# facebookresearch/D3GA

Measured on AMD Instinct MI355X. Metric: fwd+bwd frames/sec @500k Gaussians 1920x1080, higher is better.
Workload: dtype f32

## Files before the change

d3ga_amd/csrc/raster_composite_scan.hip:

```cpp
#include "composite_common.h"

#ifndef D3GA_SCAN_ABL
#define D3GA_SCAN_ABL 0
#endif
#ifndef D3GA_TILE_WAVES
#define D3GA_TILE_WAVES 4
#endif
#ifndef D3GA_TILE_PRIO
#define D3GA_TILE_PRIO 0
#endif

namespace d3ga {

#define D3GA_SCAN4(OP, BC, N) \
    OP " %0, %0, %0 row_shr:" #N " row_mask:0xf bank_mask:0xf" BC "\n" \
    OP " %1, %1, %1 row_shr:" #N " row_mask:0xf bank_mask:0xf" BC "\n" \
    OP " %2, %2, %2 row_shr:" #N " row_mask:0xf bank_mask:0xf" BC "\n" \
    OP " %3, %3, %3 row_shr:" #N " row_mask:0xf bank_mask:0xf" BC "\n"
#define D3GA_SCANX(OP, CTRL, MASK) \
    OP " %0, %0, %0 " CTRL " row_mask:" MASK " bank_mask:0xf\n" \
    OP " %1, %1, %1 " CTRL " row_mask:" MASK " bank_mask:0xf\n" \
    OP " %2, %2, %2 " CTRL " row_mask:" MASK " bank_mask:0xf\n" \
    OP " %3, %3, %3 " CTRL " row_mask:" MASK " bank_mask:0xf\n"
template <int R = 1>
__device__ __forceinline__ void row_scan_mul4(float &a, float &b, float &c, float &d) {
    asm("s_nop 1\n" D3GA_SCAN4("v_mul_f32_dpp", "", 1) D3GA_SCAN4("v_mul_f32_dpp", "", 2) D3GA_SCAN4("v_mul_f32_dpp", "", 4)
        D3GA_SCAN4("v_mul_f32_dpp", "", 8)
        : "+v"(a), "+v"(b), "+v"(c), "+v"(d));
    if constexpr (R >= 2) asm("s_nop 1\n" D3GA_SCANX("v_mul_f32_dpp", "row_bcast:15", "0xa") : "+v"(a), "+v"(b), "+v"(c), "+v"(d));
    if constexpr (R >= 4) asm("s_nop 1\n" D3GA_SCANX("v_mul_f32_dpp", "row_bcast:31", "0xc") : "+v"(a), "+v"(b), "+v"(c), "+v"(d));
}
template <int R = 1>
__device__ __forceinline__ void row_scan_add4(float &a, float &b, float &c, float &d) {
    asm("s_nop 1\n" D3GA_SCAN4("v_add_f32_dpp", " bound_ctrl:1", 1) D3GA_SCAN4("v_add_f32_dpp", " bound_ctrl:1", 2)
        D3GA_SCAN4("v_add_f32_dpp", " bound_ctrl:1", 4) D3GA_SCAN4("v_add_f32_dpp", " bound_ctrl:1", 8)
        : "+v"(a), "+v"(b), "+v"(c), "+v"(d));
    if constexpr (R >= 2) asm("s_nop 1\n" D3GA_SCANX("v_add_f32_dpp", "row_bcast:15", "0xa") : "+v"(a), "+v"(b), "+v"(c), "+v"(d));
    if constexpr (R >= 4) asm("s_nop 1\n" D3GA_SCANX("v_add_f32_dpp", "row_bcast:31", "0xc") : "+v"(a), "+v"(b), "+v"(c), "+v"(d));
}

struct ScanEntry {
    uint32_t pos, gid;
    float2 xy;
    float4 co;
    float4 rgb;
    float c2r, c2g, c2b;
};

template <bool DUAL>
__device__ __forceinline__ ScanEntry scan_gather(uint2 pg, const float2 *__restrict__ xy, const float4 *__restrict__ conic_o,
                                                 const float4 *__restrict__ rgb_invd, const float *__restrict__ colors2 ) {
    ScanEntry e;
    e.pos = pg.x; e.gid = pg.y;
    e.xy = make_float2(0.f, 0.f);
    e.co = make_float4(0.f, 0.f, 0.f, 0.f);
    e.rgb = make_float4(0.f, 0.f, 0.f, 0.f);
    e.c2r = e.c2g = e.c2b = 0.f;
    if (pg.x != 0u) {
        e.xy = xy[2 * (size_t)pg.y]; e.co = conic_o[pg.y]; e.rgb = rgb_invd[pg.y];
        if constexpr (DUAL) {
            e.c2r = colors2[3 * (size_t)pg.y]; e.c2g = colors2[3 * (size_t)pg.y + 1]; e.c2b = colors2[3 * (size_t)pg.y + 2];
        }
    }
    return e;
}

#ifdef D3GA_DIAG
__device__ unsigned long long g_diag_scan[16];
__device__ unsigned long long g_diag_waves[32768 * 4];
#endif
template <bool DUAL>
__device__ __forceinline__ void scan_consume(ScanEntry &e, uint2 &pg) {
    asm volatile("" : "+v"(e.xy.x), "+v"(e.xy.y), "+v"(e.co.x), "+v"(e.co.y), "+v"(e.co.z), "+v"(e.co.w));
    asm volatile("" : "+v"(e.rgb.x), "+v"(e.rgb.y), "+v"(e.rgb.z), "+v"(pg.x), "+v"(pg.y));
    if constexpr (DUAL) asm volatile("" : "+v"(e.c2r), "+v"(e.c2g), "+v"(e.c2b));
}

typedef float f4 __attribute__((ext_vector_type(4)));
typedef uint32_t u2 __attribute__((ext_vector_type(2)));
typedef __attribute__((address_space(3))) uint32_t lds_u32;

struct BwdArgs {
    int W, H, gx, gyv, P;
    const float2 *xy; const float4 *conic_o; const float4 *rgb_invd; const float *bg; const float *final_T; const uint32_t *n_contrib;
    const float *dL_dpix; float *acc; const float *colors2; const float *bg2; const float *dL_dpix2; const uint2 *blk_list;
    const uint32_t *blk_count; L1Source l1; const float *dL_dinvd;
    const int4 *win;
};
struct BwdDiag { unsigned long long install = 0, hit = 0, evict = 0, valid = 0, entries = 0, rowgroups = 0, trips = 0, groups = 0; };

template <bool DUAL, int S, bool INVD, int R, bool WIN>
__device__ __forceinline__ void bwd_tile_wave(const BwdArgs &A, const int tile, const uint32_t begin, const uint32_t end, const int blk,
                                              uint32_t *const s_cache, float *const s_pix, float *const s_dump, const int lane,
                                              BwdDiag &dg) {
    constexpr int PIXF = DUAL ? 12 : 8;
    constexpr int ROWF = 16 * PIXF + 4;
    constexpr int kSlot = 12;
    constexpr uint32_t kLocked = 0xffffffffu;
    constexpr int LW = 16 * R;
    const int row = lane / LW, l16 = lane & 15, lseg = lane & (LW - 1);
    constexpr int kVals = INVD ? 10 : 9, kPerInst = 64 / kVals;
    const int fq = lane / kVals, fk = lane - kVals * fq;
    const int fk_off = fk < 2 ? fk : fk + 1;
    constexpr int kAccStride = D3GA_ACC_STRIDE;
    const int bx = 2 * ((blk >> 2) & 1) + (blk & 1), by = 2 * (blk >> 3) + ((blk >> 1) & 1);
    const int tyb = tile / A.gx, view = tyb / A.gyv;
    int4 wv = make_int4(0, 0, A.W, A.H);
    if constexpr (WIN) wv = A.win[view];
    const int bx0 = (tile - tyb * A.gx) * kTile + 4 * bx + (WIN ? (wv.x & ~(kTile - 1)) : 0);
    const int by0 = (tyb - view * A.gyv) * kTile + 4 * by + (WIN ? (wv.y & ~(kTile - 1)) : 0);
    const int px = bx0 + (l16 & 3), py = by0 + (l16 >> 2);
    const bool inside = WIN ? (px >= wv.x && px < wv.x + A.W && py >= wv.y && py < wv.y + A.H) : (px < A.W && py < A.H);
    const int ix = WIN ? px - wv.x : px, iy = WIN ? py - wv.y : py;
    const size_t hw = (size_t)A.H * A.W;
    const size_t pid1 = hw * view + (size_t)iy * A.W + ix;
    const size_t pid = pid1 + 2 * hw * view;
    const float T_final = inside ? A.final_T[pid1] : 0.f;
    const uint32_t last = inside ? A.n_contrib[pid1] : 0u;
    float g0 = 0.f, g1 = 0.f, g2 = 0.f;
    if (inside && A.dL_dpix) { g0 = A.dL_dpix[pid]; g1 = A.dL_dpix[hw + pid]; g2 = A.dL_dpix[2 * hw + pid]; }
    if (inside && A.l1.image) {
        const float *tgt = A.l1.target_cell ? *A.l1.target_cell : A.l1.target;
        const float sc = A.l1.g_loss[0] * A.l1.inv_n;
        auto sgn = [](float d) { return d > 0.f ? 1.f : (d < 0.f ? -1.f : 0.f); };
        g0 += sc * sgn(A.l1.image[pid] - tgt[pid]);
        g1 += sc * sgn(A.l1.image[hw + pid] - tgt[hw + pid]);
        g2 += sc * sgn(A.l1.image[2 * hw + pid] - tgt[2 * hw + pid]);
    }
    float bg_dot = A.bg[0] * g0 + A.bg[1] * g1 + A.bg[2] * g2;
    float h0 = 0.f, h1 = 0.f, h2 = 0.f;
    if constexpr (DUAL) {
        if (inside) { h0 = A.dL_dpix2[pid]; h1 = A.dL_dpix2[hw + pid]; h2 = A.dL_dpix2[2 * hw + pid]; }
        bg_dot += A.bg2[0] * h0 + A.bg2[1] * h1 + A.bg2[2] * h2;
    }
    const uint32_t maxlast = wave_max_u32(last);
    if (maxlast == 0) return;

    float *const pixrow = s_pix + row * ROWF;
    float *const wr_base = lseg == LW - 1 ? pixrow : s_dump + 2 * lane;
    {
        float *rec = pixrow + l16 * PIXF;
        *reinterpret_cast<float4 *>(rec) = make_float4(T_final, 0.f, g0, g1);
        float gd = 0.f;
        if constexpr (INVD) gd = inside ? A.dL_dinvd[pid1] : 0.f;
        *reinterpret_cast<float4 *>(rec + 4) = make_float4(g2, T_final * bg_dot, __uint_as_float(last), gd);
        if constexpr (DUAL) *reinterpret_cast<float4 *>(rec + 8) = make_float4(h0, h1, h2, 0.f);
    }
    const uint32_t blk_cap = end - begin;
    const int qx0 = bx0 - 4 * (bx & 1), qy0 = by0 - 4 * (by & 1);
    const bool quad_in = WIN ? (qx0 < wv.x + A.W && qy0 < wv.y + A.H && qx0 + 8 > wv.x && qy0 + 8 > wv.y) : (qx0 < A.W && qy0 < A.H);
    const uint32_t cnt = quad_in ? A.blk_count[16 * (size_t)tile + blk] : 0u;
    const uint2 *const list = A.blk_list + 16 * (size_t)begin + (size_t)blk * blk_cap;
    const int ngroups = (int)((wave_max_u32(cnt) + (uint32_t)(LW - 1)) / (uint32_t)LW);
    const float ddelx_dx = 0.5f * (WIN ? wv.z : A.W), ddely_dy = 0.5f * (WIN ? wv.w : A.H);
    const float bxr = (float)bx0, byr = (float)by0;
    const int per = D3GA_SCAN_ABL == 12 ? LW : (ngroups > 0 ? ((int)cnt + ngroups - 1) / ngroups : 0);
    auto list_entry = [&](int g) -> uint2 {
        const int idx = (int)cnt - 1 - per * g - lseg;
        uint2 v = list[max(idx, 0)];
        v.x = (idx >= 0 && lseg < per) ? v.x : 0u;
        return v;
    };
    const float *const colors2v = DUAL ? A.colors2 - 3 * (size_t)view * (size_t)A.P : nullptr;
    ScanEntry e = scan_gather<DUAL>(list_entry(0), A.xy, A.conic_o, A.rgb_invd, colors2v);
    uint2 pg1 = list_entry(1);
    __builtin_amdgcn_wave_barrier();

    for (int g = 0; g < ngroups; ++g) {
        ScanEntry nxt = scan_gather<DUAL>(pg1, A.xy, A.conic_o, A.rgb_invd, colors2v);
        uint2 pg2 = list_entry(g + 2);
        const bool act = e.pos != 0u;
        const float exr = e.xy.x - bxr, eyr = e.xy.y - byr;
        const ConicQ cq = conic_q(e.co.x, e.co.y, e.co.z);
        float SA = 0.f, SB = 0.f, SC = 0.f, SyA = 0.f, SyB = 0.f, SyyA = 0.f, M6 = 0.f, M7 = 0.f, M8 = 0.f, M9 = 0.f;
#if D3GA_TILE_PRIO
        {
            const int left = ngroups - g;
            if (left > 8) __builtin_amdgcn_s_setprio(3);
            else if (left > 4) __builtin_amdgcn_s_setprio(2);
            else if (left > 2) __builtin_amdgcn_s_setprio(1);
            else __builtin_amdgcn_s_setprio(0);
        }
#endif
#pragma unroll 1
        for (int ky = 0; ky < (D3GA_SCAN_ABL == 8 ? 0 : 4); ++ky) {
            const float *const pixq = pixrow + ky * 4 * PIXF;
            float4 pa[4], pb[4], pc[4];
#pragma unroll
            for (int k = 0; k < 4; ++k) {
                pa[k] = *reinterpret_cast<const float4 *>(pixq + k * PIXF);
                pb[k] = *reinterpret_cast<const float4 *>(pixq + k * PIXF + 4);
                if constexpr (DUAL) pc[k] = *reinterpret_cast<const float4 *>(pixq + k * PIXF + 8);
                asm volatile("" : "+v"(pb[k].x), "+v"(pb[k].y), "+v"(pb[k].z));
                if constexpr (INVD) asm volatile("" : "+v"(pb[k].w));
            }
            const float dy = eyr - (float)ky;
            const float tb = cq.b * dy, tc = (cq.c * dy) * dy;
            float al[4], G[4], r[4], u[4], cgv[4], dx[4];
            bool valid[4];
#pragma unroll
            for (int k = 0; k < 4; ++k) {
                dx[k] = exr - (float)k;
                bool ok;
                splat_eval_q(dx[k], tb, tc, cq.a, e.co.w, al[k], G[k], ok);
                valid[k] = ok & (e.pos <= __float_as_uint(pb[k].z));
#ifdef D3GA_DIAG_COUNTERS
                dg.valid += valid[k] ? 1 : 0;
#endif
                al[k] = valid[k] ? al[k] : 0.f;
                r[k] = __builtin_amdgcn_rcpf(1.0f - al[k]);
                cgv[k] = e.rgb.x * pa[k].z + e.rgb.y * pa[k].w + e.rgb.z * pb[k].x;
                if constexpr (DUAL) cgv[k] += e.c2r * pc[k].x + e.c2g * pc[k].y + e.c2b * pc[k].z;
                if constexpr (INVD) cgv[k] = fmaf(e.rgb.w, pb[k].w, cgv[k]);
            }
            float p0 = r[0], p1 = r[1], p2 = r[2], p3 = r[3];
            row_scan_mul4<R>(p0, p1, p2, p3);
            const float Ti[4] = {pa[0].x * p0, pa[1].x * p1, pa[2].x * p2, pa[3].x * p3};
            float dch[4];
#pragma unroll
            for (int k = 0; k < 4; ++k) { dch[k] = al[k] * Ti[k]; u[k] = cgv[k] * dch[k]; }
            float s0 = u[0], s1 = u[1], s2 = u[2], s3 = u[3];
            row_scan_add4<R>(s0, s1, s2, s3);
            const float Sin[4] = {s0 + pa[0].y, s1 + pa[1].y, s2 + pa[2].y, s3 + pa[3].y};
            float *const wq = wr_base + ky * 4 * PIXF;
            float gop[4];
#pragma unroll
            for (int k = 0; k < 4; ++k) {
                const float dLda = Ti[k] * cgv[k] - (Sin[k] - u[k] + pb[k].y) * r[k];
                gop[k] = valid[k] ? G[k] * dLda : 0.f;
                M6 += dch[k] * pa[k].z; M7 += dch[k] * pa[k].w; M8 += dch[k] * pb[k].x;
                if constexpr (INVD) M9 = fmaf(dch[k], pb[k].w, M9);
                *reinterpret_cast<float2 *>(wq + k * PIXF) = make_float2(Ti[k], Sin[k]);
            }
            const float A = (gop[0] + gop[1]) + (gop[2] + gop[3]);
            const float B = fmaf(3.0f, gop[3], fmaf(2.0f, gop[2], gop[1]));
            const float C = fmaf(9.0f, gop[3], fmaf(4.0f, gop[2], gop[1]));
            SA += A; SB += B; SC += C;
            SyA = fmaf(dy, A, SyA); SyB = fmaf(dy, B, SyB); SyyA = fmaf(dy * dy, A, SyyA);
        }
        const float M5 = SA, ow = e.co.w;
        const float M0 = ow * (exr * SA - SB), M1 = ow * SyA;
        const float M2 = ow * (exr * (exr * SA - 2.0f * SB) + SC), M3 = ow * (exr * SyA - SyB), M4 = ow * SyyA;
        const float v0 = -(e.co.x * M0 + e.co.y * M1) * ddelx_dx;
        const float v1 = -(e.co.z * M1 + e.co.y * M0) * ddely_dy;
        const float4 va = make_float4(v0, v1, -0.5f * M2, -0.5f * M3), vb = make_float4(-0.5f * M4, M5, M6, M7);
        scan_consume<DUAL>(nxt, pg2);
        __builtin_amdgcn_wave_barrier();
        const uint32_t saddr = (uint32_t)(uintptr_t)(lds_u32 *)(s_cache + ((e.pos - 1u) & (uint32_t)(S - 1)) * kSlot);
        const uint32_t anybits = (__float_as_uint(SA) | __float_as_uint(SB) | __float_as_uint(SC)) | (__float_as_uint(SyA) | __float_as_uint(SyB) | __float_as_uint(SyyA)) |
                                 (__float_as_uint(M6) | __float_as_uint(M7) | __float_as_uint(M8) | __float_as_uint(M9));
        bool pending = D3GA_SCAN_ABL == 1 ? (anybits == 0x12345u) : (D3GA_SCAN_ABL == 8 ? act : (anybits << 1) != 0u);
#ifdef D3GA_DIAG_TIMELINE
        dg.groups += 1;
#endif
#ifdef D3GA_DIAG_COUNTERS
        dg.entries += act ? 1 : 0;
        dg.rowgroups += (act && lseg == 0) ? 1 : 0;
#endif
        while (__builtin_amdgcn_ballot_w64(pending) != 0ull) {
#ifdef D3GA_DIAG_TIMELINE
            dg.trips += 1;
#endif
            uint32_t old;
            f4 ca, cb;
            u2 cc;
            asm("" : "=v"(old), "=v"(ca), "=v"(cb), "=v"(cc));
            float c9 = 0.f;
            if constexpr (INVD) {
                asm("" : "=v"(c9));
                if (pending)
                    asm volatile("ds_wrxchg_rtn_b32 %0, %5, %6 offset:40\n"
                                 "ds_read_b128 %1, %5\n"
                                 "ds_read_b128 %2, %5 offset:16\n"
                                 "ds_read_b64 %3, %5 offset:32\n"
                                 "ds_read_b32 %4, %5 offset:44\n"
                                 "s_waitcnt lgkmcnt(0)"
                                 : "+v"(old), "+v"(ca), "+v"(cb), "+v"(cc), "+v"(c9)
                                 : "v"(saddr), "v"(kLocked)
                                 : "memory");
            } else
            if (pending)
                asm volatile("ds_wrxchg_rtn_b32 %0, %4, %5 offset:40\n"
                             "ds_read_b128 %1, %4\n"
                             "ds_read_b128 %2, %4 offset:16\n"
                             "ds_read_b64 %3, %4 offset:32\n"
                             "s_waitcnt lgkmcnt(0)"
                             : "+v"(old), "+v"(ca), "+v"(cb), "+v"(cc)
                             : "v"(saddr), "v"(kLocked)
                             : "memory");
            const bool won = pending && old != kLocked;
            const bool hit = won && old == e.pos;
            const bool evi = won && !hit && old != 0u;
#ifdef D3GA_DIAG_COUNTERS
            if (hit) dg.hit += 1; else if (evi) dg.evict += 1; else if (won) dg.install += 1;
#endif
            const f4 ta = {va.x + (hit ? ca.x : 0.f), va.y + (hit ? ca.y : 0.f), va.z + (hit ? ca.z : 0.f), va.w + (hit ? ca.w : 0.f)};
            const f4 tb4 = {vb.x + (hit ? cb.x : 0.f), vb.y + (hit ? cb.y : 0.f), vb.z + (hit ? cb.z : 0.f), vb.w + (hit ? cb.w : 0.f)};
            const u2 tc = {__float_as_uint(M8 + (hit ? __uint_as_float(cc.x) : 0.f)), e.gid};
            if constexpr (INVD) {
                const float t9 = M9 + (hit ? c9 : 0.f);
                if (won) asm volatile("ds_write_b32 %0, %1 offset:44" : : "v"(saddr), "v"(t9) : "memory");
            }
            if (won)
                asm volatile("ds_write_b128 %0, %1\n"
                             "ds_write_b128 %0, %2 offset:16\n"
                             "ds_write_b64 %0, %3 offset:32\n"
                             "ds_write_b32 %0, %4 offset:40"
                             :
                             : "v"(saddr), "v"(ta), "v"(tb4), "v"(tc), "v"(e.pos)
                             : "memory");
            pending = pending && !won;
            const unsigned long long em = __builtin_amdgcn_ballot_w64(evi);
            if (em != 0ull) {
                const int rank = lanes_below(em), total = (int)__popcll(em);
                for (int c0 = 0; c0 < total; c0 += 20) {
                    if (evi && rank >= c0 && rank < c0 + 20) {
                        float *st = s_dump + (rank - c0) * 12;
                        st[0] = ca.x; st[1] = ca.y; st[2] = ca.z; st[3] = ca.w;
                        st[4] = cb.x; st[5] = cb.y; st[6] = cb.z; st[7] = cb.w;
                        st[8] = __uint_as_float(cc.x); st[9] = c9; st[10] = __uint_as_float(cc.y);
                    }
                    const int n = min(total - c0, 20);
                    __builtin_amdgcn_wave_barrier();
                    for (int base = 0; base < n; base += kPerInst) {
                        const int ent = base + fq;
                        if (fq < kPerInst && ent < n) {
                            const float val = s_dump[ent * 12 + fk];
                            const uint32_t og = __float_as_uint(s_dump[ent * 12 + 10]);
                            if (D3GA_SCAN_ABL != 13 && val != 0.f) atomicAdd(A.acc + kAccStride * (size_t)og + fk_off, val);
                        }
                    }
                    __builtin_amdgcn_wave_barrier();
                }
            }
        }
        e = nxt;
        pg1 = pg2;
    }
}

template <bool DUAL, int S, bool INVD = false, int R = 1, bool PVB = false, bool WIN = false>
__global__ __launch_bounds__(256 * R, (DUAL ? (D3GA_TILE_WAVES < 3 ? D3GA_TILE_WAVES : 3) : D3GA_TILE_WAVES)) void composite_bwd_tile_kernel(
   
    int W, int H, int gx, int gy, int gyv, const uint32_t *__restrict__ tile_start, uint64_t dcap, const float2 *__restrict__ xy,
    const float4 *__restrict__ conic_o, const float4 *__restrict__ rgb_invd, const float *__restrict__ bg,
    const float *__restrict__ final_T, const uint32_t *__restrict__ n_contrib, const float *__restrict__ dL_dpix,
    float *__restrict__ acc, const uint32_t *__restrict__ tile_order, const float *__restrict__ colors2,
    const float *__restrict__ bg2, const float *__restrict__ dL_dpix2, const uint2 *__restrict__ blk_list,
    const uint32_t *__restrict__ blk_count, int assign, L1Source l1, const float *__restrict__ dL_dinvd, int split_cap, const uint32_t *__restrict__ split_cnt, int P,
    const int4 *__restrict__ win) {
    static_assert((S & (S - 1)) == 0, "power of two");
    constexpr int NW = 4 * R;
    constexpr int SEG = 4 / R, LW = 16 * R;
    constexpr int PIXF = DUAL ? 12 : 8;
    constexpr int ROWF = 16 * PIXF + 4;
    constexpr int kSlot = 12;
    const bool early_exit_off = (assign & 8) != 0;
    assign &= 7;
    const int tiles = gx * gy;
    int rank = (int)blockIdx.x, half = -1;
    if (R == 1 && split_cap > 0) {
        const int split_h = split_cnt ? min((int)*split_cnt, split_cap) : split_cap;
        if (rank < 2 * split_h) { half = rank & 1; rank >>= 1; } else rank -= split_h;
    }
    const int tile = tile_order ? (rank < tiles ? (int)tile_order[rank] : -1) : (rank < tiles ? rank : -1);
    if (tile < 0) return;
    const uint32_t begin = (uint32_t)min((uint64_t)tile_start[tile], dcap);
    const uint32_t end = (uint32_t)min((uint64_t)tile_start[tile + 1], dcap);
    if (begin >= end) return;

    __shared__ __attribute__((aligned(16))) float s_pix_all[NW][SEG * ROWF];
    __shared__ __attribute__((aligned(16))) float s_dump_all[NW][64 * 2 + 16 * PIXF];
    __shared__ __attribute__((aligned(16))) uint32_t s_cache[S * kSlot];
    const int nslots = min(S, (int)(end - begin));
    for (int i = threadIdx.x; i < nslots; i += 64 * NW) s_cache[i * kSlot + 10] = 0u;
    __shared__ uint32_t s_arrived;
    if (threadIdx.x == 0) s_arrived = 0u;
    __shared__ uint8_t s_perm[16];
    if (R > 1 || half >= 0) assign = 2;
    if (assign == 2 && threadIdx.x < 16) {
        int4 wv = make_int4(0, 0, W, H);
        if constexpr (WIN) wv = win[(tile / gx) / gyv];
        const int b = threadIdx.x, tx0 = (tile % gx) * kTile + (WIN ? (wv.x & ~(kTile - 1)) : 0), ty0 = ((tile / gx) % gyv) * kTile + (WIN ? (wv.y & ~(kTile - 1)) : 0);
        auto count_of = [&](int j) -> uint32_t {
            const int q = j >> 2, qx = tx0 + ((q & 1) << 3), qy = ty0 + ((q >> 1) << 3);
            const bool in = WIN ? (qx < wv.x + W && qy < wv.y + H && qx + 8 > wv.x && qy + 8 > wv.y) : (qx < W && qy < H);
            return in ? blk_count[16 * (size_t)tile + j] : 0u;
        };
        const uint32_t mine = count_of(b);
        int rank = 0;
#pragma unroll
        for (int j = 0; j < 16; ++j) {
            const uint32_t c = count_of(j);
            rank += (c > mine || (c == mine && j < b)) ? 1 : 0;
        }
        s_perm[rank] = (uint8_t)b;
    }
    __syncthreads();

    const int wave = threadIdx.x >> 6, lane = threadIdx.x & 63;
    const int row = lane / LW;
    constexpr int kVals = INVD ? 10 : 9, kPerInst = 64 / kVals;
    const int fq = lane / kVals, fk = lane - kVals * fq;
    const int fk_off = fk < 2 ? fk : fk + 1;
    constexpr int kAccStride = D3GA_ACC_STRIDE;
    float *const s_pix = s_pix_all[wave];
    float *const s_dump = s_dump_all[wave];
    BwdDiag dg;
#ifdef D3GA_DIAG_TIMELINE
    const unsigned long long diag_t0 = __builtin_readcyclecounter(), diag_w0 = __builtin_amdgcn_s_memrealtime();
#endif

    {
        int blk;
        if (assign == 2) blk = s_perm[SEG * ((wave + (int)blockIdx.x) & (NW - 1)) + row];
        else {
            const int bx = assign ? 2 * (row & 1) + (wave & 1) : 2 * (wave & 1) + (row & 1);
            const int by = assign ? 2 * (row >> 1) + (wave >> 1) : 2 * (wave >> 1) + (row >> 1);
            blk = 4 * ((bx >> 1) + 2 * (by >> 1)) + ((bx & 1) + 2 * (by & 1));
        }
        const float *const bgv = PVB ? bg + 3 * ((tile / gx) / gyv) : bg;
        const BwdArgs A = {W, H, gx, gyv, P, xy, conic_o, rgb_invd, bgv, final_T, n_contrib, dL_dpix, acc, colors2, bg2, dL_dpix2, blk_list, blk_count, l1, dL_dinvd, win};
        if (R == 1 && half >= 0) {
            blk = s_perm[2 * (2 * ((wave + (int)blockIdx.x) & 3) + (lane >> 5)) + half];
            bwd_tile_wave<DUAL, S, INVD, (R == 1 ? 2 : R), WIN>(A, tile, begin, end, blk, s_cache, s_pix, s_dump, lane, dg);
        } else
        bwd_tile_wave<DUAL, S, INVD, R, WIN>(A, tile, begin, end, blk, s_cache, s_pix, s_dump, lane, dg);
    }

#ifdef D3GA_DIAG_COUNTERS
    atomicAdd(&g_diag_scan[3], dg.install); atomicAdd(&g_diag_scan[4], dg.hit); atomicAdd(&g_diag_scan[5], dg.evict);
    atomicAdd(&g_diag_scan[8], dg.valid); atomicAdd(&g_diag_scan[9], dg.entries); atomicAdd(&g_diag_scan[10], dg.rowgroups);
#endif
#ifdef D3GA_DIAG_TIMELINE
    if (lane == 0 && dg.groups && blockIdx.x < 32768 / NW) {
        const unsigned long long diag_w1 = __builtin_amdgcn_s_memrealtime();
        const size_t slot = NW * (size_t)blockIdx.x + wave;
        g_diag_waves[4 * slot] = diag_w0 | ((__builtin_readcyclecounter() - diag_t0) << 40);
        g_diag_waves[4 * slot + 1] = diag_w1;
        g_diag_waves[4 * slot + 2] = dg.groups | (dg.trips << 16) | ((unsigned long long)(end - begin) << 32);
        g_diag_waves[4 * slot + 3] = (unsigned long long)__builtin_amdgcn_s_getreg(63492) | ((unsigned long long)(__builtin_amdgcn_s_getreg(6164) & 15) << 32);
    }
#endif
    if (D3GA_SCAN_ABL == 13 || D3GA_SCAN_ABL == 1) return;
    uint32_t arrived = 0u;
    __builtin_amdgcn_fence(__ATOMIC_RELEASE, "workgroup");
    if (lane == 0) arrived = __hip_atomic_fetch_add(&s_arrived, 1u, __ATOMIC_ACQ_REL, __HIP_MEMORY_SCOPE_WORKGROUP);
    __builtin_amdgcn_fence(__ATOMIC_ACQUIRE, "workgroup");
    arrived = (uint32_t)__builtin_amdgcn_readfirstlane((int)arrived);
    if (arrived != (uint32_t)(NW - 1) && !early_exit_off) return;
    if (early_exit_off) { __syncthreads(); if (wave != 0) return; }
    for (int base = 0; base < nslots; base += kPerInst) {
        const int ent = base + min(fq, kPerInst - 1);
        const bool mine = fq < kPerInst && ent < nslots;
        const uint32_t *const sl = s_cache + min(ent, S - 1) * kSlot;
        const uint32_t tag = sl[10], gid = sl[9];
        const float val = __uint_as_float(sl[fk < 9 ? fk : 11]);
        if (mine && tag != 0u && val != 0.f) atomicAdd(acc + kAccStride * (size_t)gid + fk_off, val);
    }
}

#ifdef D3GA_DIAG
extern "C" __attribute__((visibility("default"))) int d3ga_diag_scan_read(unsigned long long *out16, int reset) {
    if (hipMemcpyFromSymbol(out16, HIP_SYMBOL(g_diag_scan), sizeof(unsigned long long) * 16) != hipSuccess) return 1;
    if (reset) {
        unsigned long long z[16] = {0, 0, 0, 0, 0, 0, 0, 0, 0, 0, 0, 0, 0, 0, 0, 0};
        if (hipMemcpyToSymbol(HIP_SYMBOL(g_diag_scan), z, sizeof(z)) != hipSuccess) return 1;
        void *w = nullptr;
        if (hipGetSymbolAddress(&w, HIP_SYMBOL(g_diag_waves)) != hipSuccess || hipMemset(w, 0, sizeof(unsigned long long) * 4 * 32768) != hipSuccess) return 1;
    }
    return 0;
}
extern "C" __attribute__((visibility("default"))) int d3ga_diag_scan_waves(unsigned long long *out, int n) {
    return hipMemcpyFromSymbol(out, HIP_SYMBOL(g_diag_waves), sizeof(unsigned long long) * 4 * (size_t)n) != hipSuccess;
}
#endif

int launch_composite_bwd_scan(const d3ga_raster_params *prm, int gx, int gy, const BinBuf &bin, const GeomBuf &g,
                              const ImgBuf &im, int64_t d_capacity, const float *bg, const float *dL_dpix, float *acc,
                              bool ordered, const float *colors2, const float *bg2, const float *dL_dpix2, const L1Source &l1,
                              hipStream_t s, const float *dL_dinvd) {
    const uint32_t *order = ordered ? (const uint32_t *)bin.tile_order : (const uint32_t *)nullptr;
    const int split_knob = composite_bwd_split();
    const int split_cap = !ordered ? 0 : (split_knob < 0 ? (gx * gy + 9) / 10 : min(split_knob, gx * gy));
    const uint32_t *split_cnt = (ordered && split_knob < 0) ? (const uint32_t *)(bin.counters + D3GA_CNT_HEAVY) : (const uint32_t *)nullptr;
    const dim3 tgrid(gx * gy + split_cap);
    const int S = composite_merge_slots();
    const bool pvb = n_views_of(prm) > 1 && prm->per_view_background;
    const bool wnd = is_windowed(prm);
    const int4 *wtab = wnd ? win_table((void *)bin.counters, (int64_t)gx * gy, d_capacity) : nullptr;
#define D3GA_LAUNCH_TILE_R(DUALV, SV, INVDV, RV, PVBV, WINV)                                                                  \
    hipLaunchKernelGGL((composite_bwd_tile_kernel<DUALV, SV, INVDV, RV, PVBV, WINV>), tgrid, dim3(256 * RV),                    \
                       0, s, prm->W, prm->H, gx, gy, gy / n_views_of(prm), bin.tile_start, \
                       (uint64_t)d_capacity, reinterpret_cast<const float2 *>(g.xyh), g.conic_o, g.rgb_invd, bg, im.final_T, im.n_contrib, dL_dpix, acc, order,   \
                       colors2, bg2, dL_dpix2, (const uint2 *)im.blk_list, (const uint32_t *)im.blk_count, composite_tile_assign(), l1, dL_dinvd, split_cap, split_cnt, prm->P, wtab)
#define D3GA_LAUNCH_TILE(DUALV, SV, INVDV)                                                                                    \
    do {                                                                                                                      \
        if (wnd) { if (pvb) D3GA_LAUNCH_TILE_R(DUALV, SV, INVDV, 1, true, true); else D3GA_LAUNCH_TILE_R(DUALV, SV, INVDV, 1, false, true); } \
        else if (pvb) D3GA_LAUNCH_TILE_R(DUALV, SV, INVDV, 1, true, false);                                                   \
        else D3GA_LAUNCH_TILE_R(DUALV, SV, INVDV, 1, false, false);                                                           \
    } while (0)
    if (dL_dinvd) {
        if (colors2) return D3GA_E_CONFIG;
        if (S >= 512) D3GA_LAUNCH_TILE(false, 512, true); else D3GA_LAUNCH_TILE(false, 256, true);
    } else if (colors2) { if (S >= 512) D3GA_LAUNCH_TILE(true, 512, false); else D3GA_LAUNCH_TILE(true, 256, false); }
    else if (S >= 512) D3GA_LAUNCH_TILE(false, 512, false);
    else D3GA_LAUNCH_TILE(false, 256, false);
#undef D3GA_LAUNCH_TILE
#undef D3GA_LAUNCH_TILE_R
    return check_launch(s, prm->debug);
}

__global__ void row_scan_selftest_kernel(const float *__restrict__ in, float *__restrict__ out, int n) {
    const int i = blockIdx.x * blockDim.x + threadIdx.x;
    const float x = in[i];
    float a0 = x, a1 = 2.f * x, a2 = 3.f * x, a3 = 4.f * x;
    row_scan_add4(a0, a1, a2, a3);
    float m0 = 1.f + 0.125f * x, m1 = 1.f + 0.25f * x, m2 = 1.f + 0.375f * x, m3 = 1.f + 0.5f * x;
    row_scan_mul4(m0, m1, m2, m3);
    float *o = out + 8 * (size_t)i;
    o[0] = a0; o[1] = a1; o[2] = a2; o[3] = a3; o[4] = m0; o[5] = m1; o[6] = m2; o[7] = m3;
}

}

extern "C" int d3ga_selftest_row_scan(int n, const float *in, float *out, d3ga_stream_t stream) {
    if (n <= 0 || (n % 256) != 0) return D3GA_E_SIZE;
    if (!in || !out) return D3GA_E_NULL;
    hipLaunchKernelGGL(d3ga::row_scan_selftest_kernel, dim3(n / 256), dim3(256), 0, (hipStream_t)stream, in, out, n);
    return d3ga::check_launch((hipStream_t)stream, 0);
}
```

Before: 2581.

## Restructure backward scan group math and ping-pong prefetch buffers

Reworks the per-group backward composite loop. It ping-pongs two ScanEntry buffers via a lambda unrolled by two to avoid copying the prefetched entry, fully unrolls the ky loop, and hoists dx. It also folds the background term into the prefix-sum seed and rewrites the alpha gradient algebraically to drop extra per-pixel terms, and moves the opacity scaling out of the moment sums using integer-ky moments recentred by eyr. This cuts VALU work and register moves, but raises register pressure and changes numerics, for example by dividing by opacity through an approximate reciprocal.

```diff
diff --git a/d3ga_amd/csrc/raster_composite_scan.hip b/d3ga_amd/csrc/raster_composite_scan.hip
--- a/d3ga_amd/csrc/raster_composite_scan.hip
+++ b/d3ga_amd/csrc/raster_composite_scan.hip
@@ -39,30 +39,28 @@
     if constexpr (R >= 4) asm("s_nop 1\n" D3GA_SCANX("v_add_f32_dpp", "row_bcast:31", "0xc") : "+v"(a), "+v"(b), "+v"(c), "+v"(d));
 }
 
+typedef float f2 __attribute__((ext_vector_type(2)));
+typedef float f4 __attribute__((ext_vector_type(4)));
 struct ScanEntry {
     uint32_t pos, gid;
-    float2 xy;
-    float4 co;
-    float4 rgb;
+    f2 xy;
+    f4 co;
+    f4 rgb;
     float c2r, c2g, c2b;
 };
 
 template <bool DUAL>
-__device__ __forceinline__ ScanEntry scan_gather(uint2 pg, const float2 *__restrict__ xy, const float4 *__restrict__ conic_o,
-                                                 const float4 *__restrict__ rgb_invd, const float *__restrict__ colors2 ) {
-    ScanEntry e;
+__device__ __forceinline__ void scan_gather(ScanEntry &e, uint2 pg, const float2 *__restrict__ xy, const float4 *__restrict__ conic_o,
+                                            const float4 *__restrict__ rgb_invd, const float *__restrict__ colors2 ) {
     e.pos = pg.x; e.gid = pg.y;
-    e.xy = make_float2(0.f, 0.f);
-    e.co = make_float4(0.f, 0.f, 0.f, 0.f);
-    e.rgb = make_float4(0.f, 0.f, 0.f, 0.f);
-    e.c2r = e.c2g = e.c2b = 0.f;
     if (pg.x != 0u) {
-        e.xy = xy[2 * (size_t)pg.y]; e.co = conic_o[pg.y]; e.rgb = rgb_invd[pg.y];
+        e.xy = *reinterpret_cast<const f2 *>(xy + 2 * (size_t)pg.y);
+        e.co = *reinterpret_cast<const f4 *>(conic_o + pg.y);
+        e.rgb = *reinterpret_cast<const f4 *>(rgb_invd + pg.y);
         if constexpr (DUAL) {
             e.c2r = colors2[3 * (size_t)pg.y]; e.c2g = colors2[3 * (size_t)pg.y + 1]; e.c2b = colors2[3 * (size_t)pg.y + 2];
         }
     }
-    return e;
 }
 
 #ifdef D3GA_DIAG
@@ -71,12 +69,10 @@
 #endif
 template <bool DUAL>
 __device__ __forceinline__ void scan_consume(ScanEntry &e, uint2 &pg) {
-    asm volatile("" : "+v"(e.xy.x), "+v"(e.xy.y), "+v"(e.co.x), "+v"(e.co.y), "+v"(e.co.z), "+v"(e.co.w));
-    asm volatile("" : "+v"(e.rgb.x), "+v"(e.rgb.y), "+v"(e.rgb.z), "+v"(pg.x), "+v"(pg.y));
+    asm volatile("" : "+v"(e.xy), "+v"(e.co), "+v"(e.rgb), "+v"(pg.x), "+v"(pg.y));
     if constexpr (DUAL) asm volatile("" : "+v"(e.c2r), "+v"(e.c2g), "+v"(e.c2b));
 }
 
-typedef float f4 __attribute__((ext_vector_type(4)));
 typedef uint32_t u2 __attribute__((ext_vector_type(2)));
 typedef __attribute__((address_space(3))) uint32_t lds_u32;
 
@@ -140,10 +136,10 @@
     float *const wr_base = lseg == LW - 1 ? pixrow : s_dump + 2 * lane;
     {
         float *rec = pixrow + l16 * PIXF;
-        *reinterpret_cast<float4 *>(rec) = make_float4(T_final, 0.f, g0, g1);
+        *reinterpret_cast<float4 *>(rec) = make_float4(T_final, T_final * bg_dot, g0, g1);
         float gd = 0.f;
         if constexpr (INVD) gd = inside ? A.dL_dinvd[pid1] : 0.f;
-        *reinterpret_cast<float4 *>(rec + 4) = make_float4(g2, T_final * bg_dot, __uint_as_float(last), gd);
+        *reinterpret_cast<float4 *>(rec + 4) = make_float4(g2, 0.f, __uint_as_float(last), gd);
         if constexpr (DUAL) *reinterpret_cast<float4 *>(rec + 8) = make_float4(h0, h1, h2, 0.f);
     }
     const uint32_t blk_cap = end - begin;
@@ -162,17 +158,23 @@
         return v;
     };
     const float *const colors2v = DUAL ? A.colors2 - 3 * (size_t)view * (size_t)A.P : nullptr;
-    ScanEntry e = scan_gather<DUAL>(list_entry(0), A.xy, A.conic_o, A.rgb_invd, colors2v);
+    ScanEntry e0, e1;
+    e0.xy = f2{0.f, 0.f};
+    e0.co = f4{0.f, 0.f, 0.f, 0.f};
+    e0.rgb = f4{0.f, 0.f, 0.f, 0.f};
+    e0.c2r = e0.c2g = e0.c2b = 0.f;
+    scan_gather<DUAL>(e0, list_entry(0), A.xy, A.conic_o, A.rgb_invd, colors2v);
+    e1 = e0;
     uint2 pg1 = list_entry(1);
     __builtin_amdgcn_wave_barrier();
 
-    for (int g = 0; g < ngroups; ++g) {
-        ScanEntry nxt = scan_gather<DUAL>(pg1, A.xy, A.conic_o, A.rgb_invd, colors2v);
+    auto group = [&](ScanEntry &e, ScanEntry &nxt, const int g) {
+        scan_gather<DUAL>(nxt, pg1, A.xy, A.conic_o, A.rgb_invd, colors2v);
         uint2 pg2 = list_entry(g + 2);
         const bool act = e.pos != 0u;
         const float exr = e.xy.x - bxr, eyr = e.xy.y - byr;
         const ConicQ cq = conic_q(e.co.x, e.co.y, e.co.z);
-        float SA = 0.f, SB = 0.f, SC = 0.f, SyA = 0.f, SyB = 0.f, SyyA = 0.f, M6 = 0.f, M7 = 0.f, M8 = 0.f, M9 = 0.f;
+        float SA = 0.f, SB = 0.f, SC = 0.f, TyA = 0.f, TyB = 0.f, TyyA = 0.f, M6 = 0.f, M7 = 0.f, M8 = 0.f, M9 = 0.f;
 #if D3GA_TILE_PRIO
         {
             const int left = ngroups - g;
@@ -182,7 +184,10 @@
             else __builtin_amdgcn_s_setprio(0);
         }
 #endif
-#pragma unroll 1
+        float dx[4];
+#pragma unroll
+        for (int k = 0; k < 4; ++k) dx[k] = exr - (float)k;
+#pragma unroll
         for (int ky = 0; ky < (D3GA_SCAN_ABL == 8 ? 0 : 4); ++ky) {
             const float *const pixq = pixrow + ky * 4 * PIXF;
             float4 pa[4], pb[4], pc[4];
@@ -191,63 +196,67 @@
                 pa[k] = *reinterpret_cast<const float4 *>(pixq + k * PIXF);
                 pb[k] = *reinterpret_cast<const float4 *>(pixq + k * PIXF + 4);
                 if constexpr (DUAL) pc[k] = *reinterpret_cast<const float4 *>(pixq + k * PIXF + 8);
-                asm volatile("" : "+v"(pb[k].x), "+v"(pb[k].y), "+v"(pb[k].z));
+                asm volatile("" : "+v"(pb[k].x), "+v"(pb[k].z));
                 if constexpr (INVD) asm volatile("" : "+v"(pb[k].w));
             }
             const float dy = eyr - (float)ky;
             const float tb = cq.b * dy, tc = (cq.c * dy) * dy;
-            float al[4], G[4], r[4], u[4], cgv[4], dx[4];
-            bool valid[4];
+            float al[4], Gr[4], cgv[4], r4[4];
 #pragma unroll
             for (int k = 0; k < 4; ++k) {
-                dx[k] = exr - (float)k;
+                float alpha, G;
                 bool ok;
-                splat_eval_q(dx[k], tb, tc, cq.a, e.co.w, al[k], G[k], ok);
-                valid[k] = ok & (e.pos <= __float_as_uint(pb[k].z));
+                splat_eval_q(dx[k], tb, tc, cq.a, e.co.w, alpha, G, ok);
+                const float p = fmaf(dx[k], fmaf(cq.a, dx[k], tb), tc);
+                const float oG = e.co.w * G;
+                const bool valid = (p <= 0.0f) & (oG >= kAlphaMin) & (e.pos - 1u < __float_as_uint(pb[k].z));
 #ifdef D3GA_DIAG_COUNTERS
-                dg.valid += valid[k] ? 1 : 0;
-#endif
-                al[k] = valid[k] ? al[k] : 0.f;
-                r[k] = __builtin_amdgcn_rcpf(1.0f - al[k]);
+                dg.valid += valid ? 1 : 0;
+#endif
+                const float oGv = valid ? oG : 0.f;
+                al[k] = fminf(kAlphaMax, oGv);
+                const float r = __builtin_amdgcn_rcpf(1.0f - al[k]);
+                Gr[k] = oGv * r;
                 cgv[k] = e.rgb.x * pa[k].z + e.rgb.y * pa[k].w + e.rgb.z * pb[k].x;
                 if constexpr (DUAL) cgv[k] += e.c2r * pc[k].x + e.c2g * pc[k].y + e.c2b * pc[k].z;
                 if constexpr (INVD) cgv[k] = fmaf(e.rgb.w, pb[k].w, cgv[k]);
+                r4[k] = r;
             }
-            float p0 = r[0], p1 = r[1], p2 = r[2], p3 = r[3];
-            row_scan_mul4<R>(p0, p1, p2, p3);
-            const float Ti[4] = {pa[0].x * p0, pa[1].x * p1, pa[2].x * p2, pa[3].x * p3};
-            float dch[4];
-#pragma unroll
-            for (int k = 0; k < 4; ++k) { dch[k] = al[k] * Ti[k]; u[k] = cgv[k] * dch[k]; }
-            float s0 = u[0], s1 = u[1], s2 = u[2], s3 = u[3];
-            row_scan_add4<R>(s0, s1, s2, s3);
-            const float Sin[4] = {s0 + pa[0].y, s1 + pa[1].y, s2 + pa[2].y, s3 + pa[3].y};
+            row_scan_mul4<R>(r4[0], r4[1], r4[2], r4[3]);
+            float Ti[4], dch[4], s[4];
+#pragma unroll
+            for (int k = 0; k < 4; ++k) { Ti[k] = pa[k].x * r4[k]; dch[k] = al[k] * Ti[k]; s[k] = cgv[k] * dch[k]; }
+            row_scan_add4<R>(s[0], s[1], s[2], s[3]);
             float *const wq = wr_base + ky * 4 * PIXF;
             float gop[4];
 #pragma unroll
             for (int k = 0; k < 4; ++k) {
-                const float dLda = Ti[k] * cgv[k] - (Sin[k] - u[k] + pb[k].y) * r[k];
-                gop[k] = valid[k] ? G[k] * dLda : 0.f;
-                M6 += dch[k] * pa[k].z; M7 += dch[k] * pa[k].w; M8 += dch[k] * pb[k].x;
+                const float Sin = s[k] + pa[k].y;
+                gop[k] = Gr[k] * fmaf(Ti[k], cgv[k], -Sin);
+                M6 = fmaf(dch[k], pa[k].z, M6); M7 = fmaf(dch[k], pa[k].w, M7); M8 = fmaf(dch[k], pb[k].x, M8);
                 if constexpr (INVD) M9 = fmaf(dch[k], pb[k].w, M9);
-                *reinterpret_cast<float2 *>(wq + k * PIXF) = make_float2(Ti[k], Sin[k]);
+                *reinterpret_cast<float2 *>(wq + k * PIXF) = make_float2(Ti[k], Sin);
             }
             const float A = (gop[0] + gop[1]) + (gop[2] + gop[3]);
             const float B = fmaf(3.0f, gop[3], fmaf(2.0f, gop[2], gop[1]));
             const float C = fmaf(9.0f, gop[3], fmaf(4.0f, gop[2], gop[1]));
-            SA += A; SB += B; SC += C;
-            SyA = fmaf(dy, A, SyA); SyB = fmaf(dy, B, SyB); SyyA = fmaf(dy * dy, A, SyyA);
+            if (ky == 0) { SA = A; SB = B; SC = C; }
+            else { SA += A; SB += B; SC += C; }
+            if (ky == 1) { TyA = A; TyB = B; TyyA = A; }
+            if (ky >= 2) { TyA = fmaf((float)ky, A, TyA); TyB = fmaf((float)ky, B, TyB); TyyA = fmaf((float)(ky * ky), A, TyyA); }
         }
-        const float M5 = SA, ow = e.co.w;
-        const float M0 = ow * (exr * SA - SB), M1 = ow * SyA;
-        const float M2 = ow * (exr * (exr * SA - 2.0f * SB) + SC), M3 = ow * (exr * SyA - SyB), M4 = ow * SyyA;
+        const float eSA = eyr * SA;
+        const float SyA = eSA - TyA, SyB = fmaf(eyr, SB, -TyB), SyyA = fmaf(eyr, fmaf(-2.0f, TyA, eSA), TyyA);
+        const float M5 = SA * __builtin_amdgcn_rcpf(fmaxf(e.co.w, kAlphaMin));
+        const float M0 = exr * SA - SB, M1 = SyA;
+        const float M2 = exr * (exr * SA - 2.0f * SB) + SC, M3 = exr * SyA - SyB, M4 = SyyA;
         const float v0 = -(e.co.x * M0 + e.co.y * M1) * ddelx_dx;
         const float v1 = -(e.co.z * M1 + e.co.y * M0) * ddely_dy;
         const float4 va = make_float4(v0, v1, -0.5f * M2, -0.5f * M3), vb = make_float4(-0.5f * M4, M5, M6, M7);
         scan_consume<DUAL>(nxt, pg2);
         __builtin_amdgcn_wave_barrier();
         const uint32_t saddr = (uint32_t)(uintptr_t)(lds_u32 *)(s_cache + ((e.pos - 1u) & (uint32_t)(S - 1)) * kSlot);
-        const uint32_t anybits = (__float_as_uint(SA) | __float_as_uint(SB) | __float_as_uint(SC)) | (__float_as_uint(SyA) | __float_as_uint(SyB) | __float_as_uint(SyyA)) |
+        const uint32_t anybits = (__float_as_uint(SA) | __float_as_uint(SB) | __float_as_uint(SC)) | (__float_as_uint(TyA) | __float_as_uint(TyB) | __float_as_uint(TyyA)) |
                                  (__float_as_uint(M6) | __float_as_uint(M7) | __float_as_uint(M8) | __float_as_uint(M9));
         bool pending = D3GA_SCAN_ABL == 1 ? (anybits == 0x12345u) : (D3GA_SCAN_ABL == 8 ? act : (anybits << 1) != 0u);
 #ifdef D3GA_DIAG_TIMELINE
@@ -334,8 +343,12 @@
                 }
             }
         }
-        e = nxt;
         pg1 = pg2;
+    };
+    for (int g = 0; g < ngroups; g += 2) {
+        group(e0, e1, g);
+        if (g + 1 == ngroups) break;
+        group(e1, e0, g + 1);
     }
 }
 
```

Result: faster. 2631 (median of 6 runs) (+1.9%).
